# jiawei415/muzero-hypermodel

Hardware: AMD Instinct MI355X
Metric: mcts_simulations_per_sec (higher is better)
Workload: dtype f64

## Files before the change

### muzero-hypermodel_amd/build.py

```python
import os
import shutil
import subprocess

PKG_DIR = os.path.dirname(os.path.abspath(__file__))
CSRC = os.path.join(PKG_DIR, "csrc")
LIB_PATH = os.path.join(PKG_DIR, "libmzmcts.so")
SOURCES = ["mcts_kernels.hip", "fused_narrow.hip", "mzmcts_capi.hip", "mzmcts_moves.hip", "mzmcts_rng.hip", "mzhist.hip", "env_kernels.hip", "mzenv_capi.hip", "obs_stack.hip", "mzreplay.hip", "net_kernels.hip", "board_conv.hip", "wide_conv.hip", "downsample_cnn.hip", "trainer_kernels.hip", "fc_train.hip", "fc_optimizer.hip", "grad_fold.hip", "bn_epilogue.hip", "conv_train.hip", "head_train.hip", "rescale_train.hip", "device_checks.hip"]
HEADERS = ["engine_host.h", "board_rules.h", "gomoku_rules.h", "solo_rules.h", "obs_stack.h", "np_legacy_rng.h", "select_action.h", "replay_sampler.h", "replay_filer.h", "game_outcomes.h", "reanalyse_plan.h", "launch_plan.h", "wide_conv.h", "board_launch.h", "fc_net_host.h", "fc_backward.h", "fc_optimizer.h", "grad_fold.h", "bn_epilogue.h", "conv_train.h", "head_train.h", "rescale_train.h", "glibc_libm.h", "glibc_libm_tables.inc", "tree_layout.h", "tree_device.h", "fc_net_device.h", "narrow_device.h", "kernel_common.h", "env_layout.h", os.path.join("..", "..", "include", "mzmcts.h"),
           os.path.join("..", "..", "include", "mzenv.h"), os.path.join("..", "..", "include", "mzreplay.h"), os.path.join("..", "..", "include", "mzhist.h"), os.path.join("..", "..", "include", "mztrain.h")]

HIPCC_FLAGS = ["--offload-arch=gfx950", "-O3", "-std=c++17", "-fPIC", "-ffp-contract=off",
               "-fno-fast-math", "-fno-slp-vectorize", "-Wall", "-Wno-unused-variable"] + os.environ.get("MZMCTS_EXTRA_HIPCC_FLAGS", "").split()
OBJ_DIR = os.path.join(CSRC, "_obj")


def _hipcc():
    for cand in (shutil.which("hipcc"), "/opt/rocm/bin/hipcc"):
        if cand and os.path.exists(cand):
            return cand
    raise RuntimeError("hipcc not found: the MI355X MCTS engine cannot be built without ROCm")


def _obj(src):
    return os.path.join(OBJ_DIR, os.path.splitext(src)[0] + ".o")


def _flags_stamp():
    return " ".join(HIPCC_FLAGS)


def _object_deps(src):
# ... 100 lines not shown
```

### muzero-hypermodel_amd/csrc/engine_host.h

```cpp
#pragma once
#include <hip/hip_runtime.h>

#include <cmath>
#include <cstdio>
#include <cstdlib>
#include <cstring>
#include <atomic>
#include <chrono>
#include <condition_variable>
#include <functional>
#include <initializer_list>
#include <memory>
#include <mutex>
#include <string>
#include <thread>
#include <vector>

#include "../../include/mzhist.h"
#include "../../include/mzmcts.h"
#include "fc_net_device.h"
#include "kernel_common.h"
#include "narrow_device.h"
#include "np_legacy_rng.h"
#include "tree_layout.h"


namespace mz {
int default_group_width(int A);
hipError_t launch_fc_inference(const TreeParams& p, const FcNet& net, const float* weights, bool initial, const float* in,
                               const int64_t* action, float* value_logits, float* reward_logits, float* policy_logits,
                               float* hidden_out, hipStream_t stream);
size_t fc_inference_lds_bytes(const TreeParams& p, const FcNet& net);
bool plan_fused_layout(const TreeParams& p, const FcNet& net, bool want_hidden_in_lds, size_t lds_limit,
                       FusedLayout* out);
bool narrow_supported(const TreeParams& p, const FcNet& net);
bool plan_narrow_layout(const TreeParams& p, const FcNet& net, size_t lds_limit, NarrowLayout* out);
size_t narrow_table_doubles(int S, int mode);
hipError_t build_narrow_table(const TreeParams& p, int mode, double* out, hipStream_t stream);
hipError_t launch_search_fused_narrow(const TreeParams& p, const FcNet& net, const NarrowLayout& lay, const float* weights,
                                      const float* observations, const MoveCtl& ctl, int n_sims, int publish_tree,
                                      hipStream_t stream, const LaunchTiming* timing);
hipError_t launch_fc_inference_narrow(const TreeParams& p, const FcNet& net, const float* weights, bool initial,
                                      const float* in, const int64_t* action, float* value_logits, float* reward_logits,
                                      float* policy_logits, float* hidden_out, hipStream_t stream);
hipError_t launch_search_fused_fc(const TreeParams& p, const FcNet& net, const FusedLayout& lay, const float* weights,
                                  const float* observations, const MoveCtl& ctl, int n_sims, hipStream_t stream,
                                  const LaunchTiming* timing);
hipError_t launch_select(const TreeParams& p, int sim, float* hidden_out, int64_t* action_out, int queue_trees,
                         hipStream_t stream, const LaunchTiming* timing);
hipError_t launch_root_noise(const TreeParams& p, uint32_t* rng_skip, hipStream_t stream);
hipError_t launch_move_inputs(const TreeParams& p, const uint32_t* rng_skip, const uint8_t* stall, const int32_t* move_limit,
                              int move_index, bool draw_noise, int32_t* nlegal_out, int32_t* to_play_out, uint32_t* words_out,
                              int32_t* legal_out, const MoveInputsExtra& extra, hipStream_t stream);
hipError_t launch_lockstep_move_finish(const TreeParams& p, const MoveCtl& ctl, hipStream_t stream);
hipError_t launch_select_action_general(const TreeParams& p, const MoveCtl& ctl, const double* temperature,
                                        hipStream_t stream);
hipError_t launch_gather_dynamics_input(const TreeParams& p, const int64_t* action, float* out, int plane, int action_space,
                                        hipStream_t stream);
hipError_t launch_expand_roots(const TreeParams& p, const float* value_logits, const float* reward_logits,
// ... 162 lines not shown
    std::vector<uint64_t> behind;
    mz::HostStream& mirror(int e) {
        mz::HostStream& s = streams[static_cast<size_t>(e)];
        if (behind[static_cast<size_t>(e)]) {
            s.skip(behind[static_cast<size_t>(e)]);
            behind[static_cast<size_t>(e)] = 0;
        }
        return s;
    }

    std::vector<int32_t> last_visits;
    std::vector<double> last_root_value_sum;
    std::vector<int32_t> last_root_visits;

    bool fc_ready = false;
    int fused_variant = MZMCTS_FUSED_AUTO;
    bool publish_tree = true;
    bool tree_published = true;
    mz::FcNet fc{};
    const float* fc_weights = nullptr;
    bool narrow_row_rng = true;
    bool narrow_prefetch = true;
    bool narrow_generic_shape = false;
    double* narrow_table[3] = {nullptr, nullptr, nullptr};

    bool profiling = false;
    bool device_noise = false;
    bool noise_on_device = false;
    bool device_temperatures = false;
    uint32_t* h_noise_words = nullptr;
    int select_queue_trees = 0;
    std::vector<EventPair> events;
    size_t events_used = 0;
    mzmcts_profile prof{};

    std::vector<void*> device_allocs;
    std::vector<void*> pinned_allocs;

    uint8_t* h_upload = nullptr;
    uint8_t* d_upload = nullptr;
    size_t upload_bytes = 0, upload_bytes_no_noise = 0;
    uint8_t* h_download = nullptr;
    uint8_t* d_download = nullptr;
    size_t download_bytes = 0;
    bool tie_words_applied = false;

// ... 140 lines not shown
```

### muzero-hypermodel_amd/csrc/fused_narrow.hip

```cpp
#include <hip/hip_runtime.h>
#include <hip/hip_ext.h>

#include <algorithm>
#include <cstdlib>

#include "fc_net_device.h"
#include "kernel_common.h"
#include "narrow_device.h"
#include "np_legacy_rng.h"
#include "tree_device.h"
#include "tree_layout.h"

namespace mz {

constexpr int kNarrowMaxThreads = 256;

static inline int narrow_span(int A, int S) {
    if (A == 2 && S <= 254) return 2;
    int span = 4;
    while (span < A) span <<= 1;
    return span;
}

bool narrow_supported(const TreeParams& p, const FcNet& net) {
    auto one_hidden = [](const FcMlp& m) { return m.n_layers == 2 && m.layer[0].out <= kRow; };
    if (p.group != kRow || p.A > kRow || p.chunks != 1) return false;
    if (net.enc + net.A > kRow || net.obs > kRow || net.F > 2 * kRow) return false;
    if (!(net.repr.n_layers == 1 || one_hidden(net.repr))) return false;
    if (!one_hidden(net.dyn) || !one_hidden(net.reward) || !one_hidden(net.value) || !one_hidden(net.policy)) return false;
    if (p.S < 1 || p.S >= 32768) return false;
    return true;
}

bool plan_narrow_layout(const TreeParams& p, const FcNet& net, size_t lds_limit, NarrowLayout* out) {
    auto align16 = [](size_t v) { return (v + 15) / 16 * 16; };
    auto align64 = [](size_t v) { return (v + 63) / 64 * 64; };
    int rows = 4;
    if (const char* env = std::getenv("MZMCTS_NARROW_ROWS")) rows = std::max(1, std::min(4, std::atoi(env)));
    int max_mode = 2;
    if (const char* env = std::getenv("MZMCTS_NARROW_PBC2")) max_mode = std::max(0, std::min(2, std::atoi(env)));
    const size_t span = static_cast<size_t>(narrow_span(p.A, p.S));
    for (int pass = 0; pass < 2; ++pass)
    for (int mode = max_mode; mode >= 0; --mode) {
        if (mode == 2 && p.S > 63) continue;
        for (int waves = 4; waves >= 1; waves >>= 1) {
            NarrowLayout lay{};
            size_t off = 0;
            lay.off_pbc = 0;
            lay.pbc2_mode = mode;
            if (const char* env = std::getenv("MZMCTS_NARROW_EXACT_DIV")) lay.exact_division = std::atoi(env) != 0;
            off = align16(sizeof(double) * 2 * (static_cast<size_t>(p.S) + 1));
            if (mode == 2) {
                lay.off_pbc2 = static_cast<uint32_t>(off);
                off = align16(off + sizeof(double) * (static_cast<size_t>(p.S) + 1) * 64);
            } else if (mode == 1) {
                lay.off_pbc2 = static_cast<uint32_t>(off);
                off = align16(off + sizeof(double) * (static_cast<size_t>(p.S) + 1) * (static_cast<size_t>(p.S) + 2) / 2);
            } else {
                lay.off_pbc2 = 0xffffffffu;
            }
            lay.off_units = static_cast<uint32_t>(off);
            off += sizeof(float) * 4 * 4 * kRow * kNarrowUnits;
            lay.off_bias = static_cast<uint32_t>(off);
            off = align64(off + sizeof(float) * kRow * kNarrowUnits);
            lay.off_trees = static_cast<uint32_t>(off);
            size_t t = static_cast<size_t>(p.S + 1) * 32 * span;
            lay.off_side = static_cast<uint32_t>(t);
            t = align16(t + sizeof(SideStats) * static_cast<size_t>(p.S + 1) * span);
            lay.off_path = static_cast<uint32_t>(t);
            t = align16(t + sizeof(int32_t) * static_cast<size_t>(p.S));
            lay.off_hidden = static_cast<uint32_t>(t);
            t = align16(t + sizeof(float) * static_cast<size_t>(p.S + 1) * net.enc);
            lay.off_misc = static_cast<uint32_t>(t);
            t = align16(t + 4 * 2 * kRow);
            lay.off_desc = static_cast<uint32_t>(t);
            if (span == 2) t += 16 * static_cast<size_t>(p.S + 1);
            t = align64(t);
            lay.tree_bytes = static_cast<uint32_t>(t);
            lay.waves = waves;
            lay.rows = rows;
            const size_t total = off + static_cast<size_t>(waves) * rows * t;
            lay.total_bytes = static_cast<uint32_t>(total);
            if (total <= (pass == 0 ? lds_limit * waves * rows / 16 : lds_limit)) {
                *out = lay;
                return true;
            }
        }
    }
    return false;
// ... 115 lines not shown
    const bool row_rng = lay.row_rng != 0;
    uint32_t* mt_key = p.mt_key + static_cast<size_t>(e) * kMtN;
    int32_t mt_pos = 0;
    if (row_rng) {
        const uint32_t skip = prefetch ? in.skip : (ctl.rng_skip ? ctl.rng_skip[e] : 0u);
        mt_pos = mt_skip_row(mt_key, prefetch ? in.mt_pos : p.mt_pos[e], skip, j);
        if (j == 0) {
            if (skip) p.mt_pos[e] = mt_pos;
            reset_search_state(p, e, nullptr);
        }
    } else if (j == 0) {
        reset_search_state(p, e, ctl.rng_skip);
    }
    if (n_root == 0) {
        if (j == 0 && ctl.actions) ctl.actions[e] = -1;
        return;
    }
    if (row_shl1_bits(j) != ((j + 1 < kRow) ? j + 1 : 0) || row_ror_bits<1>(j) != ((j + kRow - 1) & (kRow - 1))) {
        if (j == 0) atomicOr(p.error_flag, 8);
        return;
    }

    uint8_t* region = smem + lay.off_trees + static_cast<size_t>(tree_in_block) * lay.tree_bytes;
    const LdsTreeV<SPAN> tree{region, reinterpret_cast<SideStats*>(region + lay.off_side),
                              reinterpret_cast<int32_t*>(region + lay.off_path)};
    float* hidden_lds = reinterpret_cast<float*>(region + lay.off_hidden);
    int32_t* root_action_lds = reinterpret_cast<int32_t*>(region + lay.off_misc);
    float* root_logit_lds = reinterpret_cast<float*>(region + lay.off_misc) + kRow;
    static_assert(!Shape::kFixed || SPAN == 2, "the fixed shape has two actions");
    const Shape shape(p, net);
    const int enc = shape.enc(), A = shape.actions(), F = shape.features(), support = shape.support();
    const bool two_player = shape.two_player();
    const bool wide_support = F > kRow;

    float predicted;
    {
        const float obs = prefetch ? in.obs : ((j < net.obs) ? observations[static_cast<size_t>(e) * net.obs + j] : 0.f);
        const NarrowHeads h = narrow_initial(units, bias, enc, wide_support, net.repr.n_layers == 2, obs, j);
        float unused;
        narrow_support_pair(h.value_a, h.value_b, h.value_a, h.value_b, F, support, j, predicted, unused);
        const int my_action = (j < n_root) ? (prefetch ? in.root_action : p.root_action[static_cast<size_t>(e) * A + j]) : 0;
        root_action_lds[j] = my_action;
        root_logit_lds[j] = h.policy;
        if (j < enc) hidden_lds[j] = h.norm;
        group_memory_fence();
        const bool valid = j < n_root;
        double prior[1] = {narrow_softmax(valid ? root_logit_lds[my_action] : 0.f, valid)};
        if (prefetch)
// ... 58 lines not shown
        }
        MZ_STAMP(4);
        const int k_new = sim + 1;
        if constexpr (SPAN == 2) {
            write_pair_children(tree, k_new, A, prior[0], leaf_factor, j);
            link_new_node(region + lay.off_desc, link_entry, d.depth, k_new, j);
            root_entry = window_root_entry(region + lay.off_desc, j);
        } else {
            write_children<kRow, 1>(tree, k_new, A, prior, j);
        }
        if (j < enc) hidden_lds[k_new * enc + j] = h.norm;
        MZ_STAMP(5);
        backup_row<SPAN, PBC2>(tree, round, d.depth, sim, static_cast<double>(value_f), reward_f, two_player, p.discount, mm,
                               root_value_sum, root_reward, exotic, pbc, pbc2, p.S, j);
        group_memory_fence();
        if (d.depth > max_depth) max_depth = d.depth;
        depth_sum += d.depth;
        MZ_STAMP(6);
    }

    uint32_t sample_words = 0;
    int slot = 0;
    if (ctl.temperature && row_rng) {
        const ChildLinks* root_links = tree.links(0);
        slot = device_select_action_from([&](int i) { return root_links[i].visits; }, n_root,
                                         prefetch ? narrow_move_temperature(ctl, in) : move_temperature(ctl, e),
                                         [&]() { return mt_next_row(mt_key, mt_pos, j); }, &sample_words);
    }
    if (j == 0) {
        p.root_reward[e] = root_reward;
        p.root_predicted[e] = predicted;
        p.root_value_sum[e] = root_value_sum;
        p.min_max[e] = mm;
        p.max_depth[e] = max_depth;
        p.depth_sum[e] = depth_sum;
        if (ctl.temperature) {
            if (!row_rng) {
                const ChildLinks* root_links = tree.links(0);
                slot = device_select_action([&](int i) { return root_links[i].visits; }, n_root, move_temperature(ctl, e),
                                            mt_key, &mt_pos, &sample_words);
            }
            if (ctl.actions) ctl.actions[e] = slot >= 0 ? root_action_lds[slot] : slot;
            if (ctl.game_moves) ctl.game_moves[e] += 1;
        }
        if (words | sample_words) p.mt_pos[e] = mt_pos;
        if (words) p.tie_words[e] = words;
        if (ctl.tie_words) ctl.tie_words[e] = words;
        if (ctl.sample_words) ctl.sample_words[e] = sample_words;
        if (ctl.root_value_sum) ctl.root_value_sum[e] = root_value_sum;
        if (ctl.root_predicted) ctl.root_predicted[e] = predicted;
        if (ctl.max_depth) ctl.max_depth[e] = max_depth;
        if (ctl.depth_sum) ctl.depth_sum[e] = static_cast<int32_t>(depth_sum);
    }
    if (ctl.visits && j < A) ctl.visits[static_cast<size_t>(e) * A + j] = (j < n_root) ? tree.links(0)[j].visits : 0;
    const int block_words = 2 * A;
    const int n_blocks = publish_tree ? n_sims + 1 : 1;
    for (int t = j; t < n_blocks * block_words; t += kRow) {
        const int k = t / block_words, i = t - k * block_words;
        uint4* dst = reinterpret_cast<uint4*>(p.blocks + (static_cast<size_t>(k) * p.E + e) * p.line_stride);
        if (i < A) {
            ChildStats st = tree.stats(k)[i];
            const SideStats sd = tree.side(k)[i];
            st.value_sum = tree.links(k)[i].visits > 0 ? sd.value_sum : 0.0;
            if constexpr (SPAN == 2) st.prior = sd.prior;
            *reinterpret_cast<ChildStats*>(dst + 2 * i) = st;
        } else {
            *reinterpret_cast<ChildLinks*>(dst + 2 * (i - A) + 1) = tree.links(k)[i - A];
        }
    }
    for (int t = j; t < n_blocks * enc; t += kRow) {
        const int k = t / enc, i = t - k * enc;
        p.hidden[(static_cast<size_t>(k) * p.E + e) * enc + i] = hidden_lds[t];
    }
    MZ_STAMP(7);
    MZ_STAMP_FLUSH;
}

template <bool INITIAL>
__global__ __launch_bounds__(kNarrowMaxThreads) void fc_inference_narrow_kernel(
    FcNet net, const float* __restrict__ weights, int E, const float* __restrict__ in, const int64_t* __restrict__ action,
    float* __restrict__ value_logits, float* __restrict__ reward_logits, float* __restrict__ policy_logits,
    float* __restrict__ hidden_out) {
    __shared__ float4 units[kNarrowUnits * 4 * kRow];
    __shared__ float bias[kNarrowUnits * kRow];
    stage_narrow_units(net, weights, units, bias, threadIdx.x, blockDim.x);
    __syncthreads();
    const int e = blockIdx.x * (blockDim.x / kRow) + threadIdx.x / kRow;
    const int j = threadIdx.x % kRow;
    if (e >= E) return;
    const bool wide_support = net.F > kRow;
// ... 87 lines not shown
```

### muzero-hypermodel_amd/csrc/mzmcts_capi.hip

```cpp
#include "engine_host.h"
#include "fc_net_host.h"

extern "C" {

int mzmcts_abi_version(void) { return MZMCTS_ABI_VERSION; }

const char* mzmcts_last_error(const mzmcts_engine* engine) {
    return engine ? engine->error.c_str() : g_create_error.c_str();
}

int mzmcts_create(const mzmcts_config* c, mzmcts_engine** out) {
    if (!c || !out) return fail(nullptr, MZMCTS_ERR_INVALID, "mzmcts_create: null argument");
    *out = nullptr;
    if (c->num_envs <= 0 || c->num_actions <= 0 || c->num_simulations <= 0 || c->support_size < 0 ||
        c->hidden_floats < 0)
        return fail(nullptr, MZMCTS_ERR_INVALID, "mzmcts_create: sizes must be positive");
    if (c->num_players < 1 || c->num_players > 2)
        return fail(nullptr, MZMCTS_ERR_PLAYERS, "More than two player mode not implemented.");
    if (c->num_actions > 256)
        return fail(nullptr, MZMCTS_ERR_INVALID, "mzmcts_create: at most 256 actions are supported");
    if (c->num_simulations > 32767)
        return fail(nullptr, MZMCTS_ERR_INVALID, "mzmcts_create: at most 32767 simulations are supported");
    if (c->support_size > (1 << 24))
        return fail(nullptr, MZMCTS_ERR_INVALID, "mzmcts_create: support_size above 16777216 is not supported (the "
// ... 121 lines not shown
    if ((rc = dev_alloc(eng, &eng->d_seeds, E))) return cleanup_on(rc);

    {
        std::vector<double> tab(2 * K);
        for (size_t n = 0; n < K; ++n) {
            tab[n] = std::log((static_cast<double>(n) + c->pb_c_base + 1) / c->pb_c_base) + c->pb_c_init;
            tab[K + n] = std::sqrt(static_cast<double>(n));
        }
        double* d_tab = nullptr;
        if ((rc = dev_alloc(eng, &d_tab, 2 * K))) return cleanup_on(rc);
        err = hipMemcpy(d_tab, tab.data(), sizeof(double) * 2 * K, hipMemcpyHostToDevice);
        if (err != hipSuccess) return cleanup_on(hip_fail(eng, err, "hipMemcpy(pb_c table)"));
        p.pbc_log = d_tab;
        p.pbc_sqrt = d_tab + K;
    }

    {
        const char* serial = std::getenv("MZMCTS_NARROW_SERIAL_TWIST");
        eng->narrow_row_rng = !(serial && std::atoi(serial) != 0);
        const char* no_prefetch = std::getenv("MZMCTS_NARROW_NO_PREFETCH");
        eng->narrow_prefetch = !(no_prefetch && std::atoi(no_prefetch) != 0);
        const char* generic_shape = std::getenv("MZMCTS_NARROW_GENERIC_SHAPE");
        eng->narrow_generic_shape = generic_shape && std::atoi(generic_shape) != 0;
        const char* per_launch = std::getenv("MZMCTS_NARROW_TABLE_PER_LAUNCH");
        if (!(per_launch && std::atoi(per_launch) != 0)) {
            for (int mode = 1; mode <= 2; ++mode) {
                const size_t doubles = mz::narrow_table_doubles(S, mode);
                if (doubles == 0 || doubles * sizeof(double) > kLdsPerWorkgroup) continue;
                if ((rc = dev_alloc(eng, &eng->narrow_table[mode], doubles))) return cleanup_on(rc);
                err = mz::build_narrow_table(p, mode, eng->narrow_table[mode], nullptr);
                if (err != hipSuccess) return cleanup_on(hip_fail(eng, err, "build_narrow_table"));
            }
            err = hipDeviceSynchronize();
            if (err != hipSuccess) return cleanup_on(hip_fail(eng, err, "build_narrow_table"));
        }
    }

    if ((rc = pinned_alloc(eng, &eng->h_slab0, static_cast<size_t>(E) * p.line_stride))) return cleanup_on(rc);

    eng->streams.resize(E);
    eng->behind.assign(E, 0);
    eng->lag.assign(E, 0u);
    eng->last_visits.assign(static_cast<size_t>(E) * A, 0);
    eng->last_root_value_sum.assign(E, 0.0);
    eng->last_root_visits.assign(E, 0);
    std::vector<uint32_t> seeds(E);
// ... 624 lines not shown
        MZ_HIP(eng, mz::launch_fc_inference(eng->p, eng->fc, eng->fc_weights, false, hidden, action, value_logits,
                                            reward_logits, policy_logits, hidden_out, static_cast<hipStream_t>(stream)));
    return MZMCTS_OK;
}

int64_t mzmcts_fused_lds_bytes(mzmcts_engine* eng, int32_t hidden_in_lds) {
    if (!eng || !eng->fc_ready) return 0;
    if (mzhost_use_narrow(eng)) {
        mz::NarrowLayout nl{};
        mz::plan_narrow_layout(eng->p, eng->fc, kLdsPerWorkgroup, &nl);
        return nl.total_bytes;
    }
    mz::FusedLayout lay{};
    if (!mz::plan_fused_layout(eng->p, eng->fc, hidden_in_lds != 0, kLdsPerWorkgroup, &lay)) return 0;
    return lay.total_bytes;
}

}

int mzhost_launch_fused_move(mzmcts_engine* eng, const float* observations, const mz::MoveCtl& ctl, bool hidden_in_lds,
                             hipStream_t stream) {
    if (mzhost_use_narrow(eng)) {
        mz::NarrowLayout nl{};
        mz::plan_narrow_layout(eng->p, eng->fc, kLdsPerWorkgroup, &nl);
        nl.row_rng = eng->narrow_row_rng ? 1 : 0;
        nl.prefetch = eng->narrow_prefetch ? 1 : 0;
        nl.generic_shape = eng->narrow_generic_shape ? 1 : 0;
        nl.pbc2_table = eng->narrow_table[nl.pbc2_mode];
        ProfScope scope(eng, stream, kProfFused);
        MZ_HIP(eng, mz::launch_search_fused_narrow(eng->p, eng->fc, nl, eng->fc_weights, observations, ctl, eng->p.S,
                                                   eng->publish_tree ? 1 : 0, stream, scope.get()));
        eng->tree_published = eng->publish_tree;
    } else {
        mz::FusedLayout lay{};
        if (!mz::plan_fused_layout(eng->p, eng->fc, hidden_in_lds, kLdsPerWorkgroup, &lay))
            return fail(eng, MZMCTS_ERR_INVALID, "fused search: the trees of one workgroup do not fit in 160 KB of LDS (use a "
                                                 "wider group_width or the lock-step path)");
        ProfScope scope(eng, stream, kProfFused);
        MZ_HIP(eng, mz::launch_search_fused_fc(eng->p, eng->fc, lay, eng->fc_weights, observations, ctl, eng->p.S, stream,
                                               scope.get()));
        eng->tree_published = true;
    }
    return MZMCTS_OK;
}

extern "C" {

// ... 104 lines not shown
```

### muzero-hypermodel_amd/csrc/narrow_device.h

```cpp
#pragma once
#include <hip/hip_runtime.h>

#include <type_traits>

#include "fc_net_device.h"
#include "tree_device.h"

namespace mz {

constexpr int kRow = 16;

enum NarrowUnit : int {
    kURepr0 = 0,
    kURepr1,
    kUDyn1,
    kUDyn2,
    kURew1,
    kUVal1,
    kUPol1,
    kURew2a,
    kURew2b,
    kUVal2a,
    kUVal2b,
    kUPol2,
    kNarrowUnits
};

struct NarrowLayout {
    uint32_t off_pbc;
    uint32_t off_pbc2;
    uint32_t off_units;
    uint32_t off_bias;
    uint32_t off_trees;
    uint32_t tree_bytes;
    uint32_t off_side;
    uint32_t off_path;
    uint32_t off_hidden;
    uint32_t off_misc;
    uint32_t off_desc;
    uint32_t total_bytes;
    int32_t waves;
    int32_t rows;
    int32_t pbc2_mode;
    int32_t exact_division;
    int32_t row_rng;
    const double* pbc2_table;
    int32_t prefetch;
    int32_t generic_shape;
};

struct GenericShape {
    static constexpr bool kFixed = false;
    int enc_, features_, support_, actions_;
    bool two_player_;
    __device__ __forceinline__ GenericShape(const TreeParams& p, const FcNet& net)
        : enc_(net.enc), features_(net.F), support_(net.support), actions_(p.A), two_player_(p.P == 2) {}
    __device__ __forceinline__ int enc() const { return enc_; }
    __device__ __forceinline__ int features() const { return features_; }
    __device__ __forceinline__ int support() const { return support_; }
    __device__ __forceinline__ int actions() const { return actions_; }
    __device__ __forceinline__ bool two_player() const { return two_player_; }
};
struct FlagshipShape {
    static constexpr bool kFixed = true;
    static constexpr int kEnc = 8, kFeatures = 21, kSupport = 10, kActions = 2, kPlayers = 1;
    __device__ __forceinline__ FlagshipShape(const TreeParams&, const FcNet&) {}
// ... 512 lines not shown
    float tva = exp_nonpositive(h.value_a - mv), tra = exp_nonpositive(h.reward_a - mr), tp = exp_nonpositive(packed);
    asm volatile("" : "+v"(tva), "+v"(tra), "+v"(tp));
    const float eva = tva, era = tra;
    const float trb = row_ror<8>(tp), tpol = row_ror<2>(tp);
    const float evb = in_b ? tp : 0.f, erb = in_b ? trb : 0.f;
    const float e = in_p ? tpol : 0.f;
    float sv = eva + evb, sr = era + erb;
    MZ_BUTTERFLY(kRow, kRow, (sv = sv + partner<M>(sv), sr = sr + partner<M>(sr)));
    const float iv = reciprocal_of_sum(sv), ir = reciprocal_of_sum(sr);
    const float fa = static_cast<float>(j - support), fb = static_cast<float>(kRow + j - support);
    float av = fa * (eva * iv) + fb * (evb * iv);
    float ar = fa * (era * ir) + fb * (erb * ir);
    MZ_BUTTERFLY(kRow, kRow, (av = av + partner<M>(av), ar = ar + partner<M>(ar)));
    const float y = inverse_value_transform_narrow(row_ror_into<0, 0xC>(av, ar), reciprocal);
    value = row_ror_into<8, 0xC>(y, y);
    reward = row_ror_into<8, 0x3>(y, y);
    float s = e;
    MZ_BUTTERFLY(A, A, s = s + partner<M>(s));
    prior = static_cast<double>(e * reciprocal_of_sum(s));
}

using lds_u8 = __attribute__((address_space(3))) uint8_t;
using f64x2 = double __attribute__((ext_vector_type(2)));

__device__ __forceinline__ uint32_t lds_address(const void* p) {
    return static_cast<uint32_t>(reinterpret_cast<uintptr_t>((const lds_u8*)p));
}
template <typename T>
__device__ __forceinline__ T lds_load(uint32_t address) {
    return *(const __attribute__((address_space(3))) T*)(static_cast<uintptr_t>(address));
}

struct alignas(16) SideStats {
    double value_sum;
    double prior;
};

constexpr int narrow_log2(int span) { return span == 2 ? 1 : span == 4 ? 2 : span == 8 ? 3 : 4; }

template <int SPAN>
struct LdsTreeV {
    static constexpr bool kInLds = true;
    static constexpr int kShift = narrow_log2(SPAN);
    static constexpr uint32_t kBlockStride = 32u * SPAN;
    static constexpr uint32_t kLinksOffset = 16u * SPAN;
    uint8_t* blocks;
    SideStats* side_base;
    int32_t* path;
    __device__ __forceinline__ ChildStats* stats(int k) const {
        return reinterpret_cast<ChildStats*>(blocks + (static_cast<uint32_t>(k) << (5 + kShift)));
    }
    __device__ __forceinline__ ChildLinks* links(int k) const {
        return reinterpret_cast<ChildLinks*>(blocks + (static_cast<uint32_t>(k) << (5 + kShift)) + kLinksOffset);
    }
    __device__ __forceinline__ SideStats* side(int k) const { return side_base + (k << kShift); }
    __device__ __forceinline__ void path_store(int level, int packed) const { path[level] = packed; }
    __device__ __forceinline__ int path_load(int level) const { return path[level]; }
};

struct Normalizer {
    double minimum, range, y;
    bool fast;
};

__device__ __forceinline__ Normalizer make_normalizer(const MinMax& mm, unsigned long long exotic) {
    Normalizer n;
    const bool has_range = mm.maximum > mm.minimum;
    n.minimum = has_range ? mm.minimum : 0.0;
    n.range = has_range ? mm.maximum - mm.minimum : 1.0;
    n.fast = exotic == 0ull;
    const double y0 = __builtin_amdgcn_rcp(n.range);
    const double e0 = __builtin_fma(-n.range, y0, 1.0);
    const double y1 = __builtin_fma(y0, e0, y0);
    const double e1 = __builtin_fma(-n.range, y1, 1.0);
    n.y = __builtin_fma(y1, e1, y1);
    return n;
}

__device__ __forceinline__ double normalized_value(const Normalizer& n, double v) {
    const double x = v - n.minimum;
// ... 145 lines not shown
}

__device__ __forceinline__ int window_root_entry(const uint8_t* desc, int j) {
    return lds_load<uint8_t>(lds_address(desc) + static_cast<uint32_t>(j > 0 ? j : 1));
}

__device__ __forceinline__ Descent descend_window(const LdsTreeV<2>& acc, const uint8_t* desc, int root_entry, int sim,
                                                  int n_root_children, const MinMax& mm, unsigned long long exotic,
                                                  uint32_t* mt_key, int32_t& mt_pos, uint32_t& words, bool row_rng, int j,
                                                  int group_base, int32_t* error_flag) {
    const Normalizer norm = make_normalizer(mm, exotic);
    const int h = j > 0 ? j : 1;
    const int my_level = h >= 8 ? 3 : h >= 4 ? 2 : h >= 2 ? 1 : 0;
    const bool upper_half = (group_base & 32) != 0;
    const int row_shift = group_base & 16;
    const uint32_t blocks_address = lds_address(acc.blocks);
    const uint32_t desc_lane = lds_address(desc) + static_cast<uint32_t>(h);
    const bool masked_root = n_root_children < 2;
    int depth = 0, parent = 0, slot = 0;
    int entry = root_entry;
    bool at_root = true;
    for (;;) {
        const int node = entry;
        const uint32_t block = blocks_address + (static_cast<uint32_t>(node) << 6);
        const f64x2 rec0 = lds_load<f64x2>(block), rec1 = lds_load<f64x2>(block + 16u);
        const int visits0 = lds_load<int>(block + 36u), child0 = lds_load<int>(block + 40u);
        const int visits1 = lds_load<int>(block + 52u), child1 = lds_load<int>(block + 56u);
        double n0, n1;
        normalized_pair(norm, rec0[0], rec1[0], n0, n1);
        const double score0 = rec0[1] + (visits0 > 0 ? n0 : 0.0);
        double score1 = rec1[1] + (visits1 > 0 ? n1 : 0.0);
        if (at_root && masked_root && h == 1) score1 = -INFINITY;
        const bool second = score1 > score0;
        const bool undecided = !second && !(score0 > score1);
        const bool tie = score0 == score1;
        const uint32_t winners = row_bits(__ballot(second), upper_half, row_shift);
        const uint32_t stoppers = row_bits(__ballot(undecided) | __ballot((second ? child1 : child0) < 0), upper_half, row_shift);
        const uint32_t h1 = 2u | __builtin_amdgcn_ubfe(winners, 1u, 1u);
        const uint32_t h2 = (h1 << 1) | __builtin_amdgcn_ubfe(winners, h1, 1u);
        const uint32_t h3 = (h2 << 1) | __builtin_amdgcn_ubfe(winners, h2, 1u);
        const uint32_t stop_levels = __builtin_amdgcn_ubfe(stoppers, 1u, 1u) | (__builtin_amdgcn_ubfe(stoppers, h1, 1u) << 1) |
                                     (__builtin_amdgcn_ubfe(stoppers, h2, 1u) << 2) | 8u;
        const int last = __builtin_ctz(stop_levels);
        const uint32_t h_last = h3 >> (3 - last);
        const bool on_path = static_cast<uint32_t>(h) == (h3 >> (3 - my_level)) && my_level <= last;
        const bool is_last = static_cast<uint32_t>(h) == h_last;
        if (on_path && j > 0 && !(is_last && undecided)) acc.path_store(depth + my_level, (node << 16) | (second ? 1 : 0));
        const int packed = row_or(is_last ? (node | ((child0 + 1) << 8) | ((child1 + 1) << 16) | (second ? 1 << 24 : 0) |
                                             (undecided ? 1 << 25 : 0) | (tie ? 1 << 26 : 0))
                                          : 0);
// ... 25 lines not shown
        at_root = false;
    }
    return Descent{depth, parent, slot};
}

__device__ __forceinline__ int link_fetch_path(const LdsTreeV<2>& acc, int depth, int j) {
    const int level = depth - 1 - j;
    return acc.path_load(j < 3 && level >= 0 ? level : 0);
}
__device__ __forceinline__ void link_new_node(uint8_t* desc, int entry, int depth, int k_new, int j) {
    const bool mine = j < 3 && depth - 1 - j >= 0;
    const int own = mine ? (entry & 1) << j : 0;
    const int below = row_shr1_bits(own);
    const int below2 = row_shr1_bits(below);
    const int position = (2 << j) | own | below | below2;
    if (mine) desc[((entry >> 16) << 4) + position] = static_cast<uint8_t>(k_new);
    if (j == 0)
        *reinterpret_cast<uint4*>(desc + (k_new << 4)) =
            uint4{static_cast<uint32_t>(k_new) << 8, 0u, 0u, 0u};
}

__device__ __forceinline__ void write_pair_children(const LdsTreeV<2>& acc, int k, int A, double prior, double factor, int j) {
    if (j < A) {
        acc.stats(k)[j] = ChildStats{0.0, factor * prior};
        acc.side(k)[j] = SideStats{0.0, prior};
        acc.links(k)[j] = ChildLinks{0.f, 0, -1, 0};
    }
}

template <int SPAN>
struct BackupRound {
    int base, cnt;
    bool mine, leaf;
    int packed;
    SideStats own;
    float reward;
    int visits;
    int sibling_visits, above_visits;
    double sibling_prior;
    int visits_new, parent_visits;
    double factor_own, factor_sibling;
    double visits_new_f, visits_new_reciprocal;
};

template <int SPAN>
__device__ __forceinline__ BackupRound<SPAN> backup_fetch_path(const LdsTreeV<SPAN>& acc, int depth, int base, int j) {
    BackupRound<SPAN> r{};
    r.base = base;
    r.cnt = (depth - base < kRow) ? depth - base : kRow;
    r.mine = j < r.cnt;
    r.leaf = base + j == depth - 1;
    r.packed = acc.path_load(r.mine ? base + j : base);
    if constexpr (SPAN == 2) {
        if (base > 0 && j == 0) r.above_visits = acc.path_load(base - 1);
    }
    return r;
}

template <int SPAN>
__device__ __forceinline__ void backup_fetch_records(const LdsTreeV<SPAN>& acc, BackupRound<SPAN>& r, int j) {
    const int slot = r.packed & 0xffff;
    const int kk = r.packed >> 16;
    const ChildLinks* lk = acc.links(kk) + slot;
    r.own = acc.side(kk)[slot];
    r.reward = lk->reward;
    r.visits = lk->visits;
    if constexpr (SPAN == 2) {
        r.sibling_visits = acc.links(kk)[1 - slot].visits;
        r.sibling_prior = acc.side(kk)[1 - slot].prior;
        if (r.base > 0 && j == 0) {
            const int up = r.above_visits;
            r.above_visits = acc.links(up >> 16)[up & 0xffff].visits;
        }
    }
}

template <int SPAN, int MODE>
__device__ __forceinline__ void backup_fetch_factors(BackupRound<SPAN>& r, const double* pbc, const double* pbc2, int S,
                                                     int sim, int j) {
    if (r.leaf) r.visits = 0;
    r.visits_new = r.visits + 1;
    r.visits_new_f = static_cast<double>(r.visits_new);
    r.visits_new_reciprocal = refined_reciprocal(r.visits_new_f);
    if constexpr (SPAN == 2) {
        int parent_visits = row_shr1_bits(r.visits_new);
        if (j == 0) parent_visits = r.base > 0 ? r.above_visits + 1 : sim + 1;
        r.parent_visits = parent_visits;
        if (r.mine) {
            r.factor_own = exploration_factor<MODE>(pbc, pbc2, S, parent_visits, r.visits_new);
            r.factor_sibling = exploration_factor<MODE>(pbc, pbc2, S, parent_visits, r.sibling_visits);
        }
    }
}

template <int SPAN, int MODE>
__device__ __forceinline__ void backup_row(const LdsTreeV<SPAN>& acc, const BackupRound<SPAN>& first, int depth, int sim,
                                           double value, float reward_f, bool two_player, double discount, MinMax& mm,
                                           double& root_value_sum, double root_reward, unsigned long long& exotic,
                                           const double* pbc, const double* pbc2, int S, int j) {
    const int k_new = sim + 1;
    const double root_visits = static_cast<double>(sim + 1);
    const double root_visits_reciprocal = refined_reciprocal(root_visits);
    double carry = value;
    double seen_max = -INFINITY, seen_min = INFINITY;
    double into_root = 0.0;
    bool odd = false;
    BackupRound<SPAN> r = first;
    for (;;) {
        const int cnt = r.cnt;
        const int level = r.base + j;
        const bool mine = r.mine;
        const bool leaf = r.leaf;
        const int slot = r.packed & 0xffff;
        const int kk = r.packed >> 16;
        ChildStats* st = acc.stats(kk) + slot;
        ChildLinks* lk = acc.links(kk) + slot;
        SideStats* sd = acc.side(kk) + slot;
        double vs = r.own.value_sum;
        float r_f = r.reward;
        if (leaf) {
            vs = 0.0;
            r_f = reward_f;
        }
        const double rw = static_cast<double>(r_f);
        const bool same = ((depth - (level + 1)) & 1) == 0;
        const double r_signed = two_player ? (same ? -rw : rw) : rw;
        double val = carry;
        const bool is_top = j >= cnt - 1;
        for (int s = cnt - 1; s > 0; --s) {
            const double passed = row_shl1(r_signed + discount * val);
            val = is_top ? val : passed;
        }
        const double leaving = r_signed + discount * val;
        if (mine) {
            const double vs_new = vs + ((two_player && !same) ? -val : val);
            double q = quotient_with(vs_new, r.visits_new_f, r.visits_new_reciprocal);
            if ((exotic | __ballot(leaves_plain_range(vs_new))) != 0ull) q = vs_new / r.visits_new_f;
            const double seen = rw + discount * (two_player ? -q : q);
            sd->value_sum = vs_new;
            if (leaf)
                *lk = ChildLinks{reward_f, 1, k_new, 2 * k_new};
            else
                lk->visits = r.visits_new;
            st->value_sum = seen;
            if constexpr (SPAN == 2) {
                st->prior = r.factor_own * r.own.prior;
                acc.stats(kk)[1 - slot].prior = r.factor_sibling * r.sibling_prior;
            }
            seen_max = dmax(seen_max, seen);
            seen_min = dmin(seen_min, seen);
            odd = odd || leaves_plain_range(seen);
        }
        if (r.base == 0) {
            into_root = leaving;
            break;
        }
        carry = __shfl(leaving, 0, kRow);
        r = backup_fetch_path(acc, depth, r.base - kRow, j);
        backup_fetch_records(acc, r, j);
        backup_fetch_factors<SPAN, MODE>(r, pbc, pbc2, S, sim, j);
    }
    if (j == 0) {
        double seen;
        if (!two_player) {
            root_value_sum += into_root;
        } else {
            const bool same = (depth & 1) == 0;
            root_value_sum += same ? into_root : -into_root;
        }
        double mean = quotient_with(root_value_sum, root_visits, root_visits_reciprocal);
// ... 14 lines not shown
```

Before: 871.4 million.

## Store two-action LDS trees as per-word arrays instead of 64-byte node blocks

Adds a tree image abstraction for two-action trees in LDS. By default each 16-byte word kind (child stats, links, rewards) now lives in its own array across nodes. The old 64-byte block per node stays available through an environment variable. Selection loads both children's visits and child links with one 128-bit LDS read, and backup reads them once and rewrites the child link directly. The aim is to cut LDS bank conflicts and the number of load instructions when many rows touch different nodes, at the cost of extra address arithmetic and an added field in the backup state.

Result: no change. 868.2 million (-0.4%).

```diff
diff --git a/muzero-hypermodel_amd/build.py b/muzero-hypermodel_amd/build.py
--- a/muzero-hypermodel_amd/build.py
+++ b/muzero-hypermodel_amd/build.py
@@ -6,7 +6,7 @@
 CSRC = os.path.join(PKG_DIR, "csrc")
 LIB_PATH = os.path.join(PKG_DIR, "libmzmcts.so")
 SOURCES = ["mcts_kernels.hip", "fused_narrow.hip", "mzmcts_capi.hip", "mzmcts_moves.hip", "mzmcts_rng.hip", "mzhist.hip", "env_kernels.hip", "mzenv_capi.hip", "obs_stack.hip", "mzreplay.hip", "net_kernels.hip", "board_conv.hip", "wide_conv.hip", "downsample_cnn.hip", "trainer_kernels.hip", "fc_train.hip", "fc_optimizer.hip", "grad_fold.hip", "bn_epilogue.hip", "conv_train.hip", "head_train.hip", "rescale_train.hip", "device_checks.hip"]
-HEADERS = ["engine_host.h", "board_rules.h", "gomoku_rules.h", "solo_rules.h", "obs_stack.h", "np_legacy_rng.h", "select_action.h", "replay_sampler.h", "replay_filer.h", "game_outcomes.h", "reanalyse_plan.h", "launch_plan.h", "wide_conv.h", "board_launch.h", "fc_net_host.h", "fc_backward.h", "fc_optimizer.h", "grad_fold.h", "bn_epilogue.h", "conv_train.h", "head_train.h", "rescale_train.h", "glibc_libm.h", "glibc_libm_tables.inc", "tree_layout.h", "tree_device.h", "fc_net_device.h", "narrow_device.h", "kernel_common.h", "env_layout.h", os.path.join("..", "..", "include", "mzmcts.h"),
+HEADERS = ["engine_host.h", "board_rules.h", "gomoku_rules.h", "solo_rules.h", "obs_stack.h", "np_legacy_rng.h", "select_action.h", "replay_sampler.h", "replay_filer.h", "game_outcomes.h", "reanalyse_plan.h", "launch_plan.h", "wide_conv.h", "board_launch.h", "fc_net_host.h", "fc_backward.h", "fc_optimizer.h", "grad_fold.h", "bn_epilogue.h", "conv_train.h", "head_train.h", "rescale_train.h", "glibc_libm.h", "glibc_libm_tables.inc", "tree_layout.h", "tree_image.h", "tree_device.h", "fc_net_device.h", "narrow_device.h", "kernel_common.h", "env_layout.h", os.path.join("..", "..", "include", "mzmcts.h"),
            os.path.join("..", "..", "include", "mzenv.h"), os.path.join("..", "..", "include", "mzreplay.h"), os.path.join("..", "..", "include", "mzhist.h"), os.path.join("..", "..", "include", "mztrain.h")]
 
 HIPCC_FLAGS = ["--offload-arch=gfx950", "-O3", "-std=c++17", "-fPIC", "-ffp-contract=off",
diff --git a/muzero-hypermodel_amd/csrc/engine_host.h b/muzero-hypermodel_amd/csrc/engine_host.h
--- a/muzero-hypermodel_amd/csrc/engine_host.h
+++ b/muzero-hypermodel_amd/csrc/engine_host.h
@@ -34,7 +34,7 @@
 bool plan_fused_layout(const TreeParams& p, const FcNet& net, bool want_hidden_in_lds, size_t lds_limit,
                        FusedLayout* out);
 bool narrow_supported(const TreeParams& p, const FcNet& net);
-bool plan_narrow_layout(const TreeParams& p, const FcNet& net, size_t lds_limit, NarrowLayout* out);
+bool plan_narrow_layout(const TreeParams& p, const FcNet& net, size_t lds_limit, NarrowLayout* out, bool blocks_image = false);
 size_t narrow_table_doubles(int S, int mode);
 hipError_t build_narrow_table(const TreeParams& p, int mode, double* out, hipStream_t stream);
 hipError_t launch_search_fused_narrow(const TreeParams& p, const FcNet& net, const NarrowLayout& lay, const float* weights,
@@ -243,6 +243,7 @@
     bool narrow_row_rng = true;
     bool narrow_prefetch = true;
     bool narrow_generic_shape = false;
+    bool narrow_blocks_image = false;
     double* narrow_table[3] = {nullptr, nullptr, nullptr};
 
     bool profiling = false;
diff --git a/muzero-hypermodel_amd/csrc/fused_narrow.hip b/muzero-hypermodel_amd/csrc/fused_narrow.hip
--- a/muzero-hypermodel_amd/csrc/fused_narrow.hip
+++ b/muzero-hypermodel_amd/csrc/fused_narrow.hip
@@ -32,7 +32,7 @@
     return true;
 }
 
-bool plan_narrow_layout(const TreeParams& p, const FcNet& net, size_t lds_limit, NarrowLayout* out) {
+bool plan_narrow_layout(const TreeParams& p, const FcNet& net, size_t lds_limit, NarrowLayout* out, bool blocks_image) {
     auto align16 = [](size_t v) { return (v + 15) / 16 * 16; };
     auto align64 = [](size_t v) { return (v + 63) / 64 * 64; };
     int rows = 4;
@@ -65,6 +65,12 @@
             off = align64(off + sizeof(float) * kRow * kNarrowUnits);
             lay.off_trees = static_cast<uint32_t>(off);
             size_t t = static_cast<size_t>(p.S + 1) * 32 * span;
+            if (span == 2) {
+                static_assert(kPairWords * kPairWordBytes == 32 * 2, "either image of a two-action tree fills 64 bytes a node");
+                const PairImage image = blocks_image ? pair_image_blocks() : pair_image_arrays(static_cast<uint32_t>(p.S) + 1);
+                lay.tree_node_shift = image.node_shift;
+                lay.tree_word_stride = image.word_stride;
+            }
             lay.off_side = static_cast<uint32_t>(t);
             t = align16(t + sizeof(SideStats) * static_cast<size_t>(p.S + 1) * span);
             lay.off_path = static_cast<uint32_t>(t);
@@ -226,8 +232,12 @@
     }
 
     uint8_t* region = smem + lay.off_trees + static_cast<size_t>(tree_in_block) * lay.tree_bytes;
-    const LdsTreeV<SPAN> tree{region, reinterpret_cast<SideStats*>(region + lay.off_side),
-                              reinterpret_cast<int32_t*>(region + lay.off_path)};
+    const LdsTreeV<SPAN> tree = [&]() {
+        SideStats* side = reinterpret_cast<SideStats*>(region + lay.off_side);
+        int32_t* path = reinterpret_cast<int32_t*>(region + lay.off_path);
+        if constexpr (SPAN == 2) return LdsTreeV<2>{region, side, path, PairImage{lay.tree_node_shift, lay.tree_word_stride}};
+        else return LdsTreeV<SPAN>{region, side, path};
+    }();
     float* hidden_lds = reinterpret_cast<float*>(region + lay.off_hidden);
     int32_t* root_action_lds = reinterpret_cast<int32_t*>(region + lay.off_misc);
     float* root_logit_lds = reinterpret_cast<float*>(region + lay.off_misc) + kRow;
@@ -332,8 +342,7 @@
     uint32_t sample_words = 0;
     int slot = 0;
     if (ctl.temperature && row_rng) {
-        const ChildLinks* root_links = tree.links(0);
-        slot = device_select_action_from([&](int i) { return root_links[i].visits; }, n_root,
+        slot = device_select_action_from([&](int i) { return tree.load_visits(0, i); }, n_root,
                                          prefetch ? narrow_move_temperature(ctl, in) : move_temperature(ctl, e),
                                          [&]() { return mt_next_row(mt_key, mt_pos, j); }, &sample_words);
     }
@@ -346,8 +355,7 @@
         p.depth_sum[e] = depth_sum;
         if (ctl.temperature) {
             if (!row_rng) {
-                const ChildLinks* root_links = tree.links(0);
-                slot = device_select_action([&](int i) { return root_links[i].visits; }, n_root, move_temperature(ctl, e),
+                slot = device_select_action([&](int i) { return tree.load_visits(0, i); }, n_root, move_temperature(ctl, e),
                                             mt_key, &mt_pos, &sample_words);
             }
             if (ctl.actions) ctl.actions[e] = slot >= 0 ? root_action_lds[slot] : slot;
@@ -362,7 +370,7 @@
         if (ctl.max_depth) ctl.max_depth[e] = max_depth;
         if (ctl.depth_sum) ctl.depth_sum[e] = static_cast<int32_t>(depth_sum);
     }
-    if (ctl.visits && j < A) ctl.visits[static_cast<size_t>(e) * A + j] = (j < n_root) ? tree.links(0)[j].visits : 0;
+    if (ctl.visits && j < A) ctl.visits[static_cast<size_t>(e) * A + j] = (j < n_root) ? tree.load_visits(0, j) : 0;
     const int block_words = 2 * A;
     const int n_blocks = publish_tree ? n_sims + 1 : 1;
     for (int t = j; t < n_blocks * block_words; t += kRow) {
@@ -371,11 +379,11 @@
         if (i < A) {
             ChildStats st = tree.stats(k)[i];
             const SideStats sd = tree.side(k)[i];
-            st.value_sum = tree.links(k)[i].visits > 0 ? sd.value_sum : 0.0;
+            st.value_sum = tree.load_visits(k, i) > 0 ? sd.value_sum : 0.0;
             if constexpr (SPAN == 2) st.prior = sd.prior;
             *reinterpret_cast<ChildStats*>(dst + 2 * i) = st;
         } else {
-            *reinterpret_cast<ChildLinks*>(dst + 2 * (i - A) + 1) = tree.links(k)[i - A];
+            *reinterpret_cast<ChildLinks*>(dst + 2 * (i - A) + 1) = tree.load_links(k, i - A);
         }
     }
     for (int t = j; t < n_blocks * enc; t += kRow) {
diff --git a/muzero-hypermodel_amd/csrc/mzmcts_capi.hip b/muzero-hypermodel_amd/csrc/mzmcts_capi.hip
--- a/muzero-hypermodel_amd/csrc/mzmcts_capi.hip
+++ b/muzero-hypermodel_amd/csrc/mzmcts_capi.hip
@@ -1,3 +1,5 @@
+#include <cstring>
+
 #include "engine_host.h"
 #include "fc_net_host.h"
 
@@ -167,6 +169,8 @@
         eng->narrow_prefetch = !(no_prefetch && std::atoi(no_prefetch) != 0);
         const char* generic_shape = std::getenv("MZMCTS_NARROW_GENERIC_SHAPE");
         eng->narrow_generic_shape = generic_shape && std::atoi(generic_shape) != 0;
+        const char* tree_image = std::getenv("MZMCTS_NARROW_TREE_IMAGE");
+        eng->narrow_blocks_image = tree_image && std::strcmp(tree_image, "blocks") == 0;
         const char* per_launch = std::getenv("MZMCTS_NARROW_TABLE_PER_LAUNCH");
         if (!(per_launch && std::atoi(per_launch) != 0)) {
             for (int mode = 1; mode <= 2; ++mode) {
@@ -837,7 +841,7 @@
                              hipStream_t stream) {
     if (mzhost_use_narrow(eng)) {
         mz::NarrowLayout nl{};
-        mz::plan_narrow_layout(eng->p, eng->fc, kLdsPerWorkgroup, &nl);
+        mz::plan_narrow_layout(eng->p, eng->fc, kLdsPerWorkgroup, &nl, eng->narrow_blocks_image);
         nl.row_rng = eng->narrow_row_rng ? 1 : 0;
         nl.prefetch = eng->narrow_prefetch ? 1 : 0;
         nl.generic_shape = eng->narrow_generic_shape ? 1 : 0;
diff --git a/muzero-hypermodel_amd/csrc/narrow_device.h b/muzero-hypermodel_amd/csrc/narrow_device.h
--- a/muzero-hypermodel_amd/csrc/narrow_device.h
+++ b/muzero-hypermodel_amd/csrc/narrow_device.h
@@ -5,6 +5,7 @@
 
 #include "fc_net_device.h"
 #include "tree_device.h"
+#include "tree_image.h"
 
 namespace mz {
 
@@ -42,6 +43,7 @@
     int32_t waves;
     int32_t rows;
     int32_t pbc2_mode;
+    uint32_t tree_node_shift, tree_word_stride;
     int32_t exact_division;
     int32_t row_rng;
     const double* pbc2_table;
@@ -600,6 +602,7 @@
 
 using lds_u8 = __attribute__((address_space(3))) uint8_t;
 using f64x2 = double __attribute__((ext_vector_type(2)));
+using i32x4 = int __attribute__((ext_vector_type(4)));
 
 __device__ __forceinline__ uint32_t lds_address(const void* p) {
     return static_cast<uint32_t>(reinterpret_cast<uintptr_t>((const lds_u8*)p));
@@ -634,6 +637,69 @@
     __device__ __forceinline__ SideStats* side(int k) const { return side_base + (k << kShift); }
     __device__ __forceinline__ void path_store(int level, int packed) const { path[level] = packed; }
     __device__ __forceinline__ int path_load(int level) const { return path[level]; }
+    __device__ __forceinline__ ChildStats* stat(int k, int c) const { return stats(k) + c; }
+    __device__ __forceinline__ int load_visits(int k, int c) const { return links(k)[c].visits; }
+    __device__ __forceinline__ ChildLinks load_links(int k, int c) const { return links(k)[c]; }
+};
+
+template <>
+struct LdsTreeV<2> {
+    static constexpr bool kInLds = true;
+    static constexpr int kShift = 1;
+    uint8_t* blocks;
+    SideStats* side_base;
+    int32_t* path;
+    PairImage image;
+    struct StatsView {
+        uint8_t* word0;
+        uint32_t stride;
+        __device__ __forceinline__ ChildStats& operator[](int c) const {
+            return *reinterpret_cast<ChildStats*>(word0 + (c ? stride : 0u));
+        }
+    };
+    struct LinksRef {
+        int32_t* visits_child;
+        float* reward;
+        __device__ __forceinline__ void operator=(const ChildLinks& l) const {
+            *reward = l.reward;
+            *reinterpret_cast<int2*>(visits_child) = int2{l.visits, l.child_node};
+        }
+    };
+    struct LinksView {
+        uint8_t* links_word;
+        uint8_t* rewards_word;
+        __device__ __forceinline__ LinksRef operator[](int c) const {
+            return LinksRef{reinterpret_cast<int32_t*>(links_word) + 2 * c, reinterpret_cast<float*>(rewards_word) + c};
+        }
+    };
+    __device__ __forceinline__ uint8_t* word(int k, uint32_t w) const {
+        return blocks + pair_word_offset(image, static_cast<uint32_t>(k), w);
+    }
+    __device__ __forceinline__ StatsView stats(int k) const { return StatsView{word(k, kPairWordStats), image.word_stride}; }
+    __device__ __forceinline__ LinksView links(int k) const {
+        return LinksView{word(k, kPairWordLinks), word(k, kPairWordRewards)};
+    }
+    __device__ __forceinline__ SideStats* side(int k) const { return side_base + (k << kShift); }
+    __device__ __forceinline__ void path_store(int level, int packed) const { path[level] = packed; }
+    __device__ __forceinline__ int path_load(int level) const { return path[level]; }
+    __device__ __forceinline__ ChildStats* stat(int k, int c) const {
+        return reinterpret_cast<ChildStats*>(blocks + pair_stats_offset(image, static_cast<uint32_t>(k), static_cast<uint32_t>(c)));
+    }
+    __device__ __forceinline__ int32_t* visits(int k, int c) const {
+        return reinterpret_cast<int32_t*>(blocks + pair_visits_offset(image, static_cast<uint32_t>(k), static_cast<uint32_t>(c)));
+    }
+    __device__ __forceinline__ float* reward(int k, int c) const {
+        return reinterpret_cast<float*>(blocks + pair_reward_offset(image, static_cast<uint32_t>(k), static_cast<uint32_t>(c)));
+    }
+    __device__ __forceinline__ int load_visits(int k, int c) const { return *visits(k, c); }
+    __device__ __forceinline__ ChildLinks load_links(int k, int c) const {
+        const int2 vc = *reinterpret_cast<const int2*>(visits(k, c));
+        return ChildLinks{*reward(k, c), vc.x, vc.y, vc.y > 0 ? 2 * vc.y : 0};
+    }
+    __device__ __forceinline__ void store_links(int k, int c, float reward_f, int visits_new, int child_node) const {
+        *reward(k, c) = reward_f;
+        *reinterpret_cast<int2*>(visits(k, c)) = int2{visits_new, child_node};
+    }
 };
 
 struct Normalizer {
@@ -825,10 +891,10 @@
     bool at_root = true;
     for (;;) {
         const int node = entry;
-        const uint32_t block = blocks_address + (static_cast<uint32_t>(node) << 6);
-        const f64x2 rec0 = lds_load<f64x2>(block), rec1 = lds_load<f64x2>(block + 16u);
-        const int visits0 = lds_load<int>(block + 36u), child0 = lds_load<int>(block + 40u);
-        const int visits1 = lds_load<int>(block + 52u), child1 = lds_load<int>(block + 56u);
+        const uint32_t word0 = blocks_address + pair_word_offset(acc.image, static_cast<uint32_t>(node), kPairWordStats);
+        const f64x2 rec0 = lds_load<f64x2>(word0), rec1 = lds_load<f64x2>(word0 + acc.image.word_stride);
+        const i32x4 lk = lds_load<i32x4>(word0 + kPairWordLinks * acc.image.word_stride);
+        const int visits0 = lk[0], child0 = lk[1], visits1 = lk[2], child1 = lk[3];
         double n0, n1;
         normalized_pair(norm, rec0[0], rec1[0], n0, n1);
         const double score0 = rec0[1] + (visits0 > 0 ? n0 : 0.0);
@@ -900,7 +966,7 @@
 
 __device__ __forceinline__ void write_pair_children(const LdsTreeV<2>& acc, int k, int A, double prior, double factor, int j) {
     if (j < A) {
-        acc.stats(k)[j] = ChildStats{0.0, factor * prior};
+        *acc.stat(k, j) = ChildStats{0.0, factor * prior};
         acc.side(k)[j] = SideStats{0.0, prior};
         acc.links(k)[j] = ChildLinks{0.f, 0, -1, 0};
     }
@@ -915,6 +981,7 @@
     float reward;
     int visits;
     int sibling_visits, above_visits;
+    int child;
     double sibling_prior;
     int visits_new, parent_visits;
     double factor_own, factor_sibling;
@@ -939,17 +1006,22 @@
 __device__ __forceinline__ void backup_fetch_records(const LdsTreeV<SPAN>& acc, BackupRound<SPAN>& r, int j) {
     const int slot = r.packed & 0xffff;
     const int kk = r.packed >> 16;
-    const ChildLinks* lk = acc.links(kk) + slot;
     r.own = acc.side(kk)[slot];
-    r.reward = lk->reward;
-    r.visits = lk->visits;
     if constexpr (SPAN == 2) {
-        r.sibling_visits = acc.links(kk)[1 - slot].visits;
+        const i32x4 lk = *reinterpret_cast<const i32x4*>(acc.word(kk, kPairWordLinks));
+        r.reward = *acc.reward(kk, slot);
+        r.visits = slot ? lk[2] : lk[0];
+        r.child = slot ? lk[3] : lk[1];
+        r.sibling_visits = slot ? lk[0] : lk[2];
         r.sibling_prior = acc.side(kk)[1 - slot].prior;
         if (r.base > 0 && j == 0) {
             const int up = r.above_visits;
-            r.above_visits = acc.links(up >> 16)[up & 0xffff].visits;
-        }
+            r.above_visits = acc.load_visits(up >> 16, up & 0xffff);
+        }
+    } else {
+        const ChildLinks* lk = acc.links(kk) + slot;
+        r.reward = lk->reward;
+        r.visits = lk->visits;
     }
 }
 
@@ -991,8 +1063,7 @@
         const bool leaf = r.leaf;
         const int slot = r.packed & 0xffff;
         const int kk = r.packed >> 16;
-        ChildStats* st = acc.stats(kk) + slot;
-        ChildLinks* lk = acc.links(kk) + slot;
+        ChildStats* st = acc.stat(kk, slot);
         SideStats* sd = acc.side(kk) + slot;
         double vs = r.own.value_sum;
         float r_f = r.reward;
@@ -1016,14 +1087,19 @@
             if ((exotic | __ballot(leaves_plain_range(vs_new))) != 0ull) q = vs_new / r.visits_new_f;
             const double seen = rw + discount * (two_player ? -q : q);
             sd->value_sum = vs_new;
-            if (leaf)
-                *lk = ChildLinks{reward_f, 1, k_new, 2 * k_new};
-            else
-                lk->visits = r.visits_new;
+            if constexpr (SPAN == 2) {
+                acc.store_links(kk, slot, r_f, r.visits_new, leaf ? k_new : r.child);
+            } else {
+                ChildLinks* lk = acc.links(kk) + slot;
+                if (leaf)
+                    *lk = ChildLinks{reward_f, 1, k_new, 2 * k_new};
+                else
+                    lk->visits = r.visits_new;
+            }
             st->value_sum = seen;
             if constexpr (SPAN == 2) {
                 st->prior = r.factor_own * r.own.prior;
-                acc.stats(kk)[1 - slot].prior = r.factor_sibling * r.sibling_prior;
+                acc.stat(kk, 1 - slot)->prior = r.factor_sibling * r.sibling_prior;
             }
             seen_max = dmax(seen_max, seen);
             seen_min = dmin(seen_min, seen);
diff --git a/muzero-hypermodel_amd/csrc/tree_image.h b/muzero-hypermodel_amd/csrc/tree_image.h
--- /dev/null
+++ b/muzero-hypermodel_amd/csrc/tree_image.h
@@ -0,0 +1,43 @@
+#pragma once
+#include <cstdint>
+
+#if defined(__HIPCC__) || defined(__CUDACC__)
+#define MZ_TREE_IMAGE_HD __host__ __device__ inline
+#else
+#define MZ_TREE_IMAGE_HD inline
+#endif
+
+namespace mz {
+
+struct PairImage {
+    uint32_t node_shift;
+    uint32_t word_stride;
+};
+
+constexpr uint32_t kPairWordStats = 0;
+constexpr uint32_t kPairWordLinks = 2;
+constexpr uint32_t kPairWordRewards = 3;
+constexpr uint32_t kPairWords = 4;
+constexpr uint32_t kPairWordBytes = 16;
+
+MZ_TREE_IMAGE_HD PairImage pair_image_arrays(uint32_t nodes) { return PairImage{4u, kPairWordBytes * nodes}; }
+MZ_TREE_IMAGE_HD PairImage pair_image_blocks() { return PairImage{6u, kPairWordBytes}; }
+MZ_TREE_IMAGE_HD uint32_t pair_image_bytes(uint32_t nodes) { return kPairWords * kPairWordBytes * nodes; }
+
+MZ_TREE_IMAGE_HD uint32_t pair_word_offset(PairImage im, uint32_t k, uint32_t word) {
+    return (k << im.node_shift) + word * im.word_stride;
+}
+MZ_TREE_IMAGE_HD uint32_t pair_stats_offset(PairImage im, uint32_t k, uint32_t child) {
+    return pair_word_offset(im, k, kPairWordStats) + (child ? im.word_stride : 0u);
+}
+MZ_TREE_IMAGE_HD uint32_t pair_visits_offset(PairImage im, uint32_t k, uint32_t child) {
+    return pair_word_offset(im, k, kPairWordLinks) + 8u * child;
+}
+MZ_TREE_IMAGE_HD uint32_t pair_child_offset(PairImage im, uint32_t k, uint32_t child) {
+    return pair_word_offset(im, k, kPairWordLinks) + 8u * child + 4u;
+}
+MZ_TREE_IMAGE_HD uint32_t pair_reward_offset(PairImage im, uint32_t k, uint32_t child) {
+    return pair_word_offset(im, k, kPairWordRewards) + 4u * child;
+}
+
+}
```
